# centreborelli/sat-bundleadjust

Hardware: AMD Instinct MI355X
Metric: LM iters/sec at 200 cams x 1M pts x 10M obs (affine, R+T) (higher is better)
Workload: dtype f64; 1 GPU; C4: 200 cams x 1000000 pts x 9998866 obs, affine, correction R+T, 1 fixed camera, seed 1; obs_per_rank0=9998866

## Files before the change

### sat-bundleadjust_amd/csrc/satba_capi.hip

```cpp
#include <hip/hip_runtime.h>

#include <algorithm>
#include <atomic>
#include <chrono>
#include <cmath>
#include <cstdarg>
#include <cstdio>
#include <cstdlib>
#include <cstring>
#include <new>
#include <string>
#include <thread>
#include <vector>

#include "../../include/satba.h"
#include "satba_chol.h"
#include "satba_kernels.h"
#include "satba_layout.h"
#include "satba_lm.h"
#include "satba_lmdev.h"
#include "satba_outliers.h"
#include "satba_triangulate.h"
#include "satba_tracks.h"
#include "satba_ftracks.h"
// ... 51 lines not shown
constexpr int RED_SLOTS = 8, RED_MAX_GRID = 2048, RED_MAX_NV = 4;
struct SchurItems { int2* items = nullptr; SchurItem* desc = nullptr; int n_blocks = 0; };
static_assert(sizeof(SchurItemKey) == sizeof(int2) && offsetof(SchurItemKey, pair) == offsetof(int2, x) && offsetof(SchurItemKey, chunk) == offsetof(int2, y), "uploaded as int2");

struct satba_problem {
    int model = 0, M = 0, N = 0, NP = 0, c_p = 0, n_cam_fix = 0, n_pts_fix = 0, rank = 0, world = 1, f32 = 0, device = 0;
    long long K = 0, n_total = 0;
    int n_c = 0, n = 0, hdr = 0;
    int loss = 0;
    int camc_lds = 0, rpc_lds = 0;
    int cam_sums_lds = 1;
    int lin_rep_shift = 0;
    int deterministic = 0;
    int split_env = -1;
    double *d_fx = nullptr, *d_bbox = nullptr, *d_fxcost = nullptr, *d_fxcost_new = nullptr, *d_fxcost0 = nullptr;
    int *d_fxflag = nullptr, *d_fxe = nullptr;
    bool fxcost_valid = false, fxcost_new_valid = false, fxcost0_valid = false;
    double w_max = 1.0, n_max_cam = 1.0, fx_shrink = 1.0;
    int fx_fallbacks = 0;
    bool scales_by_tail = false;
    bool prep_fused = false;
    struct LmDev* d_lm = nullptr;
    struct LmSummary* h_lm = nullptr;
    struct LmSummary* h_lm_dev = nullptr;
    long long lm_ticks_queued = 0;
    hipStream_t own_stream = nullptr;
    double f_scale = 1.0, lead = 1.0;
    hipStream_t stream = nullptr;
    Layout L;
    int unit_weights = 0;
    double *d_cam_static = nullptr, *d_rpc = nullptr;
    double *d_x = nullptr, *d_xnew = nullptr, *d_camc = nullptr, *d_camc_new = nullptr;
    double *d_scale_inv = nullptr, *d_g = nullptr, *d_gh = nullptr, *d_gn = nullptr, *d_q1 = nullptr, *d_wv = nullptr;
    double *d_U = nullptr, *d_gc = nullptr, *d_V = nullptr, *d_Vinv = nullptr, *d_PV = nullptr, *d_dc = nullptr, *d_dch = nullptr;
    double2 *d_f = nullptr, *d_ftmp = nullptr;
    bool f_valid = false;
    bool prof_lin = false;
    std::vector<hipEvent_t> prof_ev;
    size_t prof_used = 0;
    double* d_Jpm = nullptr;
    double *d_part = nullptr, *d_part3 = nullptr, *d_pair_part = nullptr;
    SchurItems items_chunked;
    SchurItems items_merged;
    double2* d_W = nullptr;
    SchurItems items_w;
    int lin_grid = 0, cm_chunks = 1, cm_chunks_w = 1;
    double* d_red = nullptr;
    unsigned* d_red_cnt = nullptr;
    double* d_stage = nullptr;
    size_t stage_len = 0;
    int* d_fail = nullptr;
    double* d_dinv = nullptr;
    CholWork chol;
    bool s_scaled = false;
    hipStream_t chol_stream = nullptr;
    hipEvent_t ev_fork = nullptr, ev_join = nullptr;
    int* d_arrive = nullptr;
    int* d_pair_cnt = nullptr;
    int* d_dg_cnt = nullptr;
    long long* d_ts = nullptr;
    int msg_epoch = 0;
    double* msg_packed = nullptr;
    bool beside_last = false;
    bool beside_off = false;
    int beside_clean = 0;
    int beside_retry_after = 64;
    int beside_timeouts = 0;
    double* d_scal = nullptr;
    double* d_keep = nullptr;
    bool prepared = false;
    double *d_xb_own = nullptr, *d_xb = nullptr;
    long long xb_len = 0;
    double* h_pin = nullptr;
    bool dir_global = false;
    double* d_dir_tab = nullptr;
    void* h_stage = nullptr;
    size_t h_stage_len = 0;
    struct CopyLane { char* pin = nullptr; hipEvent_t ev[2] = {nullptr, nullptr}; };
    CopyLane lanes[8];
    hipStream_t copy_stream = nullptr;
    bool lanes_ready = false;
    double* d_err_keep = nullptr;
    hipEvent_t ev_err = nullptr;
    double* d_x0 = nullptr;
    bool linearized = false, have_step = false;
    double create_ms[8] = {0, 0, 0, 0, 0, 0, 0, 0};
    std::vector<void*> allocs;

    double* payload() const { return d_xb + hdr; }
    RedBuf red(int slot) const { return RedBuf{d_red + (size_t)slot * RED_MAX_NV * RED_MAX_GRID, d_red_cnt + slot}; }
};
struct PhaseCtx {
    const int* gate = nullptr;
    const double *Delta_dev = nullptr, *coef_dev = nullptr, *lam_force_dev = nullptr, *sub_args_dev = nullptr;
    const int* first_dev = nullptr;
    int fuse_prep = -1;
    bool skip_lin_scales = false;
    bool decide1a_in_trial = false;
    bool decide2_in_trial = false;
};
struct FrontCtx {
    int arrive_epoch = 0;
// ... 264 lines not shown
    CamMajor cm = cam_major(p);
    SATBA_DISPATCH(p, hipLaunchKernelGGL((k_cam_sums<MODEL, NP>), dim3(p->M, p->cm_chunks), dim3(LINC_THREADS), 0, p->stream, a, cm, p->d_f, p->d_part3));
    HIP_TRY(hipGetLastError());
    const int total = p->M * cam_acc_len(p->NP);
    hipLaunchKernelGGL(k_cam_sums_finish, dim3((total + 255) / 256), dim3(256), 0, p->stream, p->M, p->NP, p->cm_chunks, p->d_part3, U, gc, gate);
    HIP_TRY(hipGetLastError());
    return 0;
}

namespace {
struct SchurRoute;
int schur_items_build(satba_problem* p, SchurTable kind, SchurItems* t, long long dg_weight);
int schur_item_tables(satba_problem* p);
template <int MODEL, int NP> int launch_schur(satba_problem* p, const FrontCtx& f, const SchurRoute& r, const ObsArgs& a, double* S, double* rhs);
}
static int launch_schur_kernel(satba_problem* p, const int* gate, const FrontCtx& f, const SchurRoute& r) {
    ObsArgs a = obs_args(p, false, gate);
    double* S = p->payload();
    double* rhs = S + (size_t)p->n_c * p->n_c;
    SATBA_DISPATCH(p, TRY((launch_schur<MODEL, NP>(p, f, r, a, S, rhs))));
    return 0;
}

static int launch_backsub_kernel(satba_problem* p, const int* gate) {
    ObsArgs a = obs_args(p, false, gate);
    a.sh = slice_split(p);
    a.rev = slice_rev(1);
    const int grid = slice_grid(p, BS_THREADS / 64, 2, a.sh);
    const size_t lds = p->model == AFFINE ? dir_table_bytes(p) : table_bytes(p);
    if (p->dir_global) {
        SATBA_DISPATCH(p, if constexpr (MODEL == AFFINE) {
            hipLaunchKernelGGL((k_affine_dir_tab<NP>), dim3(1), dim3(1024), 0, p->stream, a, p->d_dc, (const double*)nullptr, (const double*)nullptr);
            hipLaunchKernelGGL((k_backsub<MODEL, NP, CL, RL, true>), dim3(grid), dim3(BS_THREADS), 0, p->stream, a, p->d_dc, p->d_dch, p->lead,
                               p->d_Vinv, p->d_g, p->d_scale_inv, p->d_gh, p->d_gn, p->red(RB_BS), p->d_xb);
        });
    } else
    SATBA_DISPATCH(p, hipLaunchKernelGGL((k_backsub<MODEL, NP, CL, RL>), dim3(grid), dim3(BS_THREADS), lds, p->stream, a, p->d_dc, p->d_dch, p->lead,
                                         p->d_Vinv, p->d_g, p->d_scale_inv, p->d_gh, p->d_gn, p->red(RB_BS), p->d_xb));
    HIP_TRY(hipGetLastError());
    return 0;
}

static int launch_jvp(satba_problem* p, const int* gate, int nv, const double* q1, const double* q2, double* out, bool pre = false) {
    ObsArgs a = obs_args(p, false, gate);
    a.sh = slice_split(p);
    a.rev = slice_rev(2);
    const int grid = slice_grid(p, JVP_THREADS / 64, 2, a.sh);
    const RedBuf rb = p->red(RB_JVP);
    if (p->dir_global && (nv == 2 || pre)) {
        SATBA_DISPATCH(p, if constexpr (MODEL == AFFINE) {
            hipLaunchKernelGGL((k_affine_dir_tab<NP>), dim3(1), dim3(1024), 0, p->stream, a, q1, nv == 2 ? q2 : nullptr, nv == 2 ? p->d_scale_inv : nullptr);
            if (nv == 1) hipLaunchKernelGGL((k_jvp<MODEL, NP, 1, CL, RL, true, true>), dim3(grid), dim3(JVP_THREADS), 0, p->stream, a, q1, q2, p->d_scale_inv, rb, out);
            else hipLaunchKernelGGL((k_jvp<MODEL, NP, 2, CL, RL, false, true>), dim3(grid), dim3(JVP_THREADS), 0, p->stream, a, q1, q2, p->d_scale_inv, rb, out);
        });
    } else if (nv == 1 && pre) {
        const size_t lds = p->model == AFFINE ? dir_table_bytes(p) : table_bytes(p);
        SATBA_DISPATCH(p, hipLaunchKernelGGL((k_jvp<MODEL, NP, 1, CL, RL, true>), dim3(grid), dim3(JVP_THREADS), lds, p->stream, a, q1, q2, p->d_scale_inv, rb, out));
    } else if (nv == 1) {
        SATBA_DISPATCH(p, hipLaunchKernelGGL((k_jvp<MODEL, NP, 1, CL, RL, false>), dim3(grid), dim3(JVP_THREADS), table_bytes(p), p->stream, a, q1, q2,
                                             p->d_scale_inv, rb, out));
    } else {
        const size_t lds = p->model == AFFINE ? std::max(table_bytes(p), 2 * dir_table_bytes(p)) : table_bytes(p);
        SATBA_DISPATCH(p, hipLaunchKernelGGL((k_jvp<MODEL, NP, 2, CL, RL, false>), dim3(grid), dim3(JVP_THREADS), lds, p->stream, a, q1, q2,
                                             p->d_scale_inv, rb, out));
    }
    HIP_TRY(hipGetLastError());
    return 0;
}

static int dense_solve(satba_problem* p, const int* gate, double* S, double* b, bool cleared = false, bool* unscaled = nullptr) {
    TrsvTail tail;
// ... 284 lines not shown
    if (const char* ss = getenv("SATBA_SPLIT")) p->split_env = atoi(ss);

    int rc = [&]() -> int {
        HIP_TRY(hipSetDevice(p->device));
        HIP_TRY(hipStreamCreateWithFlags(&p->own_stream, hipStreamNonBlocking));
        p->stream = p->own_stream;
        if (p->n_c > CH_NB * CH_MAX_STEPS) return fail(SATBA_E_ARG, "reduced camera system too large for the dense solver");
        cholesky_init();
        TRY(build_layout(p, d));
        const size_t budget = 150 * 1024;
        const size_t camc_b = sizeof(double) * (size_t)p->M * CAMC, rpc_b = sizeof(double) * (size_t)p->M * RPCS;
        while (p->lin_rep_shift < 4 && (p->M << (p->lin_rep_shift + 1)) <= 1024 &&
               cam_sum_bytes(p->NP, (size_t)(p->M << (p->lin_rep_shift + 1))) + camc_b <= 140 * 1024)
            ++p->lin_rep_shift;
        if (const char* rs = getenv("SATBA_LIN_REP")) p->lin_rep_shift = std::min(4, std::max(0, atoi(rs)));
        const size_t acc_b = cam_sum_bytes(p->NP, (size_t)(p->M << p->lin_rep_shift));
        p->cam_sums_lds = (acc_b <= budget && !p->deterministic && !getenv("SATBA_CAM_SUMS") && p->n_max_cam <= (double)FX_MAX_OBS_PER_CAM) ? 1 : 0;
        size_t used = p->cam_sums_lds ? acc_b : 0;
        p->camc_lds = (camc_b <= 48 * 1024 && used + camc_b <= budget && !getenv("SATBA_CAMC_GLOBAL")) ? 1 : 0;
        used += p->camc_lds ? camc_b : 0;
        p->rpc_lds = (p->model == RPC && rpc_b <= 64 * 1024 && used + rpc_b <= budget && !getenv("SATBA_RPC_GLOBAL")) ? 1 : 0;
        p->dir_global = p->model == AFFINE && (2 * dir_table_bytes(p) > budget || getenv("SATBA_DIR_GLOBAL"));
        if (p->dir_global) TRY(dev_alloc(p, &p->d_dir_tab, (size_t)2 * p->M * JVP_ROW));
        SATBA_DISPATCH(p, TRY((raise_lin_limits<MODEL, NP, CL, RL>(p))));

        const size_t n = p->n, Pz = (size_t)std::max(p->L.P, 1) + 64;
        TRY(dev_alloc(p, &p->d_cam_static, (size_t)p->M * p->c_p));
        if (p->model == RPC) TRY(dev_alloc(p, &p->d_rpc, (size_t)p->M * SATBA_RPC_TABLE_LEN));
        TRY(dev_alloc(p, &p->d_x, n)); TRY(dev_alloc(p, &p->d_xnew, n)); TRY(dev_alloc(p, &p->d_scale_inv, n));
        TRY(dev_alloc(p, &p->d_g, n)); TRY(dev_alloc(p, &p->d_gh, n)); TRY(dev_alloc(p, &p->d_gn, n));
        TRY(dev_alloc(p, &p->d_q1, n)); TRY(dev_alloc(p, &p->d_wv, n));
        TRY(dev_alloc(p, &p->d_camc, (size_t)p->M * CAMC)); TRY(dev_alloc(p, &p->d_camc_new, (size_t)p->M * CAMC));
        TRY(dev_alloc(p, &p->d_U, (size_t)p->M * p->NP * p->NP)); TRY(dev_alloc(p, &p->d_gc, p->n_c));
        TRY(dev_alloc(p, &p->d_V, (size_t)6 * p->N)); TRY(dev_alloc(p, &p->d_Vinv, (size_t)6 * p->N));
        TRY(dev_alloc(p, &p->d_PV, (size_t)PV_STRIDE * (p->N + 1)));
        HIP_TRY(hipMemset(p->d_PV + (size_t)PV_STRIDE * p->N, 0, sizeof(double) * PV_STRIDE));
        TRY(dev_alloc(p, &p->d_dc, p->n_c)); TRY(dev_alloc(p, &p->d_dch, p->n_c));
        const size_t Kz = (size_t)std::max<long long>(K, 1) + 64;
        TRY(dev_alloc(p, &p->d_f, Pz)); TRY(dev_alloc(p, &p->d_ftmp, Pz));
        if (p->model == RPC) TRY(dev_alloc(p, &p->d_Jpm, Kz * jrow_stride(p->NP)));
        TRY(dev_alloc(p, &p->d_fail, 1 + CH_MAX_STEPS));
        TRY(dev_alloc(p, &p->d_dinv, (size_t)((p->n_c + CH_NB - 1) / CH_NB) * CH_NB * CH_NB));
        {
            const size_t T = (size_t)(p->n_c + 63) / 64;
            TRY(dev_alloc(p, &p->chol.flags, T * T + 1)); TRY(dev_alloc(p, &p->chol.Linv, T * 4096 + 1)); TRY(dev_alloc(p, &p->chol.Cc, T * T * 64 + 1));
            TRY(dev_alloc(p, &p->chol.ctr, 4));
            HIP_TRY(hipMemset(p->chol.flags, 0, sizeof(int) * (T * T + 1)));
            HIP_TRY(hipMemset(p->chol.ctr, 0, sizeof(int) * 4));
        }
        TRY(dev_alloc(p, &p->d_scal, 8));
        TRY(dev_alloc(p, &p->d_fx, fx_scales_len(p->NP))); TRY(dev_alloc(p, &p->d_fxe, fx_exps_len(p->NP)));
        TRY(dev_alloc(p, &p->d_bbox, 6)); TRY(dev_alloc(p, &p->d_fxflag, 1));
        TRY(dev_alloc(p, &p->d_fxcost, 1)); TRY(dev_alloc(p, &p->d_fxcost_new, 1)); TRY(dev_alloc(p, &p->d_fxcost0, 1));
        HIP_TRY(hipMemset(p->d_bbox, 0, sizeof(double) * 6));
        HIP_TRY(hipMemset(p->d_fxflag, 0, sizeof(int)));
        if (const char* fs = getenv("SATBA_FX_SHRINK")) p->fx_shrink = atof(fs);
        TRY(dev_alloc(p, &p->d_lm, 1));
        HIP_TRY(hipMemset(p->d_lm, 0, sizeof(LmDev)));
        HIP_TRY(hipHostMalloc((void**)&p->h_lm, sizeof(LmSummary) + sizeof(LmDev), hipHostMallocMapped));
        memset(p->h_lm, 0, sizeof(LmSummary) + sizeof(LmDev));
        HIP_TRY(hipHostGetDevicePointer((void**)&p->h_lm_dev, p->h_lm, 0));
        TRY(dev_alloc(p, &p->d_keep, SATBA_KEEP_LEN));
        HIP_TRY(hipMemset(p->d_keep, 0, sizeof(double) * SATBA_KEEP_LEN));
        TRY(dev_alloc(p, &p->d_red, (size_t)RED_SLOTS * RED_MAX_NV * RED_MAX_GRID));
        TRY(dev_alloc(p, &p->d_red_cnt, RED_SLOTS));
        HIP_TRY(hipMemset(p->d_red_cnt, 0, sizeof(unsigned) * RED_SLOTS));
        p->lin_grid = lin_grid_for(p);
        TRY(dev_alloc(p, &p->d_part, (size_t)512 * p->M * cam_sum_len(p->NP)));
        {
            int chunks = 8;
            while (chunks < 64 && (long long)p->M * chunks < 512 && K / ((long long)p->M * (chunks + 8)) >= 4096) chunks += 8;
            while (chunks > 1 && K / ((long long)p->M * chunks) < 256) --chunks;
            int chunks_w = chunks;
            if (chunks >= 8) {
                chunks_w = std::min(64, 2 * chunks);
                while (chunks_w > chunks && K / ((long long)p->M * chunks_w) < 512) chunks_w -= 8;
            }
            if (const char* dc = getenv("SATBA_CM_CHUNKS")) chunks_w = chunks = std::max(1, std::min(256, atoi(dc)));
            p->cm_chunks = chunks; p->cm_chunks_w = chunks_w;
            TRY(dev_alloc(p, &p->d_part3, (size_t)p->M * std::max(64, std::max(chunks, chunks_w)) * (cam_acc_len(p->NP) + p->NP)));
        }
        if (p->L.C > 1) TRY(dev_alloc(p, &p->d_pair_part, (size_t)p->L.C * std::max<long long>(p->L.n_pairs, 1) * p->NP * p->NP));
        TRY(schur_item_tables(p));
        p->stage_len = std::max<size_t>(std::max<size_t>(n, 2 * (size_t)K), (size_t)6 * p->N) + 16;
        TRY(dev_alloc(p, &p->d_stage, p->stage_len));
        p->xb_len = satba_exchange_len(p);
        TRY(dev_alloc(p, &p->d_xb_own, p->xb_len));
        p->d_xb = p->d_xb_own;
        HIP_TRY(hipHostMalloc((void**)&p->h_pin, sizeof(double) * (p->hdr + 64)));
        HIP_TRY(hipMemset(p->d_xb, 0, sizeof(double) * p->xb_len));
        HIP_TRY(hipMemset(p->d_scale_inv, 0, sizeof(double) * n));
        HIP_TRY(hipMemset(p->d_x, 0, sizeof(double) * n));
        HIP_TRY(hipMemset(p->d_xnew, 0, sizeof(double) * n));
        HIP_TRY(hipMemcpy(p->d_cam_static, d->cam_params, sizeof(double) * p->M * p->c_p, hipMemcpyHostToDevice));
        if (p->model == RPC)
            HIP_TRY(hipMemcpy(p->d_rpc, d->rpc_tables, sizeof(double) * p->M * SATBA_RPC_TABLE_LEN, hipMemcpyHostToDevice));
// ... 698 lines not shown
```

### sat-bundleadjust_amd/csrc/satba_kernels.h

```cpp
#pragma once
#include <hip/hip_runtime.h>
#include <stdint.h>

#include "../../include/satba.h"
#include "satba_models.h"

namespace satba {

__host__ __device__ constexpr int cam_acc_len(int np) { return np * (np + 1) / 2 + np; }
__host__ __device__ constexpr int cam_acc_stride(int np) { return cam_acc_len(np) | 1; }
__host__ __device__ constexpr int cam_sum_len(int np) { return 3 * np; }
__host__ __device__ constexpr int cam_sum_stride(int np) { return (3 * np) | 1; }
constexpr int FX_LO_SHIFT = 40;
constexpr long long FX_MAX_OBS_PER_CAM = 1ll << 23;
__host__ __device__ constexpr size_t cam_sum_bytes(int np, size_t rows) { return (rows * cam_sum_stride(np) * 8 + 15) & ~(size_t)15; }
__host__ __device__ constexpr int fx_scales_len(int np) { return 2 * np; }
__host__ __device__ constexpr int fx_exps_len(int np) { return np + 3; }

constexpr int RPCS = 94;
static_assert(RPCS >= 90 && RPCS % 2 == 0 && (RPCS / 2) % 2 == 1, "RPC rows in the LDS: an odd number of 16-byte slots");
constexpr double FX_MAGIC = 6755399441055744.0;
constexpr unsigned long long FX_MAGIC_BITS = 0x4338000000000000ull;
__host__ __device__ constexpr int jrow_stride(int) { return 8; }

// ... 1226 lines not shown
    __syncthreads();
    if (tid < hdr_len) xb[tid] = 0.0;
    if (s_k[2] != 0.0) return;
    if (first_dev) first = *first_dev;
    double s_gh = 0.0, s_xs = 0.0, m_gc = 0.0;
    for (int i = tid; i < n_c; i += 1024) {
        const int cam = i / NP, k = i % NP;
        const double diag = payload[(size_t)cam * NP * NP + k * NP + k], gi = payload[nU + i];
        g[i] = gi;
        m_gc = fmax(m_gc, fabs(gi));
        double si = sqrt(diag);
        if (first) si = (si == 0.0) ? 1.0 : si;
        else si = fmax(si, scale_inv[i]);
        scale_inv[i] = si;
        const double h = gi / si;
        gh[i] = h;
        ghs[i] = h / si;
        s_gh += lead * h * h;
        const double xs = x[i] * si;
        s_xs += lead * xs * xs;
    }
    s_gh = wave_sum(s_gh); s_xs = wave_sum(s_xs); m_gc = wave_max(m_gc);
    if (lane == 0) { s_red[0][wave] = s_gh; s_red[1][wave] = s_xs; s_red[2][wave] = m_gc; }
    __syncthreads();
    if (tid == 0) {
        double a = 0.0, b = 0.0, m = 0.0;
        for (int w = 0; w < 16; ++w) { a += s_red[0][w]; b += s_red[1][w]; m = fmax(m, s_red[2][w]); }
        xb[SATBA_HDR_GH_SQ] = a + s_k[0];
        xb[SATBA_HDR_XS_SQ] = b + s_k[1];
        xb[SATBA_HDR_GC_INF] = lead * m;
    }
}

#ifndef SATBA_BS_THREADS
#define SATBA_BS_THREADS 512
#endif
constexpr int BS_THREADS = SATBA_BS_THREADS;
template <int MODEL, int NP, bool CL, bool RL, bool DG = false>
__global__ __launch_bounds__(BS_THREADS) void k_backsub(ObsArgs a, const double* __restrict__ dc, const double* __restrict__ dch,
                                                        double lead, const double* __restrict__ Vinv, const double* __restrict__ g,
                                                        const double* __restrict__ scale_inv, const double* __restrict__ gh,
                                                        double* __restrict__ gn, RedBuf rb, double* __restrict__ hdr) {
    SATBA_GATE(a.gate);
    extern __shared__ __attribute__((aligned(16))) double s_dyn_bs[];
    const int lane = threadIdx.x & 63;
    constexpr int WAVES = BS_THREADS / 64;
    double sa = 0.0, sb = 0.0, sc = 0.0;
    if (blockIdx.x == 0) {
        for (int i = threadIdx.x; i < a.n_c; i += BS_THREADS) {
            const double v = dch[i], h = gh[i];
            gn[i] = v;
            sa += lead * h * h; sb += lead * h * v; sc += lead * v * v;
        }
    }
    CamTables<CL, RL> T;
    const double* tab = DG ? a.dir_tab : s_dyn_bs;
    if constexpr (MODEL == AFFINE) { if constexpr (!DG) affine_dir_table<NP>(a, dc, s_dyn_bs, BS_THREADS); }
    else T.stage(a, s_dyn_bs, BS_THREADS);
    for_each_slice(a.n_slices << a.sh, WAVES, [&](const int u) {
        const SliceUnit su(a, u, lane);
        const int q = su.q;
        const bool has = q < a.N;
        const int cnt = has ? a.pt_cnt[q] : 0;
        double X = 0.0, Y = 0.0, Z = 0.0, mp = 0.0;
        if (has) {
            const double* px = a.x + a.n_c + 3 * (size_t)q;
            X = px[0]; Y = px[1]; Z = px[2];
            mp = (a.perm[q] >= a.n_pts_fix) ? 1.0 : 0.0;
        }
        double t[3] = {0.0, 0.0, 0.0};
        int pos = su.pos;
        const int io0 = has ? a.ipt_ofs[q] : 0;
        if constexpr (MODEL == AFFINE) {
            constexpr int D = SATBA_CAM_PF;
// ... 20 lines not shown
                    DirRow R;
                    R.load(tab, cam);
                    const double* row = R.v;
                    const double u0 = mp * s2.x * s2.x * (row[0] * X + row[1] * Y + row[2] * Z + row[6]);
                    const double u1 = mp * s2.y * s2.y * (row[3] * X + row[4] * Y + row[5] * Z + row[7]);
#pragma unroll
                    for (int j = 0; j < 3; ++j) t[j] += row[8 + j] * u0 + row[11 + j] * u1;
                }
            }
        } else {
            for (int tt = 0; tt < su.nt; ++tt, pos += su.step) {
                const int k = su.slot(tt);
                if (k < cnt) {
                    const int cam = a.e_cam[pos];
                    ObsEval<MODEL, NP, true> e;
                    e.jac(a, io0 + k, cam, mp, T.cc(cam), T.tab(cam), X, Y, Z);
                    double u0 = 0.0, u1 = 0.0;
#pragma unroll
                    for (int i = 0; i < NP; ++i) {
                        const double d = dc[cam * NP + i];
                        u0 += e.Jc[0][i] * d;
                        u1 += e.Jc[1][i] * d;
                    }
#pragma unroll
                    for (int j = 0; j < 3; ++j) t[j] += e.Jp[0][j] * u0 + e.Jp[1][j] * u1;
                }
            }
        }
        if (su.sh) {
#pragma unroll
            for (int j = 0; j < 3; ++j) t[j] = slice_point_sum(t[j], su.sh);
        }
        if (has && su.g == 0) {
            const double* vi = Vinv + 6 * (size_t)q;
            const size_t ib = (size_t)a.n_c + 3 * (size_t)q;
            const double r0 = g[ib] - t[0], r1 = g[ib + 1] - t[1], r2 = g[ib + 2] - t[2];
            const double d[3] = {vi[0] * r0 + vi[1] * r1 + vi[2] * r2, vi[1] * r0 + vi[3] * r1 + vi[4] * r2,
                                 vi[2] * r0 + vi[4] * r1 + vi[5] * r2};
#pragma unroll
            for (int k = 0; k < 3; ++k) {
                const double v = d[k] * scale_inv[ib + k], h = gh[ib + k];
                gn[ib + k] = v;
                sa += h * h; sb += h * v; sc += v * v;
            }
        }
    }, a.rev);
    double v[3] = {sa, sb, sc};
    double* const dst[3] = {hdr + SATBA_HDR_GRAM_A, hdr + SATBA_HDR_GRAM_B, hdr + SATBA_HDR_GRAM_C};
    grid_sum<3>(v, dst, rb);
}

__global__ __launch_bounds__(256) void k_subspace_vec(int n, int n_c, double lead, double alpha, double s,
                                                      const double* __restrict__ gh, const double* __restrict__ gn,
                                                      double* __restrict__ q1, double* __restrict__ wv, RedBuf rb,
                                                      double* __restrict__ hdr, const double* __restrict__ args_dev, const int* gate) {
    SATBA_GATE(gate);
    if (args_dev) { alpha = args_dev[0]; s = args_dev[1]; }
    double ww = 0.0, wq = 0.0, gw = 0.0;
    for (int i = blockIdx.x * blockDim.x + threadIdx.x; i < n; i += gridDim.x * blockDim.x) {
        const double h = gh[i], q = s * h, w = gn[i] - alpha * h;
        q1[i] = q;
        wv[i] = w;
        const double wgt = (i < n_c) ? lead : 1.0;
        ww += wgt * w * w; wq += wgt * w * q; gw += wgt * h * w;
    }
    double v[3] = {ww, wq, gw};
    double* const dst[3] = {hdr + SATBA_HDR_WW, hdr + SATBA_HDR_WQ1, hdr + SATBA_HDR_GHW};
    grid_sum<3>(v, dst, rb);
// ... 20 lines not shown
```

### sat-bundleadjust_amd/csrc/satba_schur.h

```cpp
#pragma once
#include "satba_kernels.h"

namespace satba {

constexpr int PV_STRIDE = 16;
__device__ inline double schur_lambda(const double* __restrict__ hdr, double Delta, double lam_floor, double* __restrict__ keep, bool write) {
    const double gh_sq = hdr[SATBA_HDR_GH_SQ], jg_sq = hdr[SATBA_HDR_JG_SQ], xs_sq = hdr[SATBA_HDR_XS_SQ];
    if (!(Delta > 0.0)) {
        Delta = sqrt(xs_sq);
        if (Delta == 0.0) Delta = 1.0;
    }
    const double a = 0.5 * jg_sq, b = -gh_sq, ub = Delta / sqrt(gh_sq);
    double best = fmin(0.0, a * ub * ub + b * ub);
    if (a != 0.0) {
        const double ext = -0.5 * b / a;
        if (0.0 < ext && ext < ub) best = fmin(best, a * ext * ext + b * ext);
    }
    double lam = -best / (Delta * Delta);
    if (!(lam >= lam_floor)) lam = lam_floor;
    if (write) {
        keep[SATBA_KEEP_GINF] = fmax(keep[SATBA_KEEP_GINF], hdr[SATBA_HDR_GC_INF]);
        keep[SATBA_KEEP_GH_SQ] = gh_sq; keep[SATBA_KEEP_JG_SQ] = jg_sq; keep[SATBA_KEEP_XS_SQ] = xs_sq;
        keep[SATBA_KEEP_LAM] = lam;
        keep[SATBA_KEEP_DELTA] = Delta;
    }
    return lam;
}

#ifndef SATBA_VINV_THREADS
#define SATBA_VINV_THREADS 256
#endif
constexpr int VINV_THREADS = SATBA_VINV_THREADS;
__global__ __launch_bounds__(VINV_THREADS) void k_vinv(int N, double lam, const double* __restrict__ hdr_auto, double Delta, double lam_floor,
                                                       double* __restrict__ keep, const double* __restrict__ V,
                                                       const double* __restrict__ scale_inv_p, double* __restrict__ Vinv,
                                                       const double* __restrict__ xp, const double* __restrict__ gp, double* __restrict__ PV,
                                                       const int* __restrict__ perm, int n_pts_fix, const double* __restrict__ Delta_dev,
                                                       const double* __restrict__ lam_force, const int* gate, const int* __restrict__ w_fix = nullptr) {
    SATBA_GATE(gate);
    if (Delta_dev) Delta = *Delta_dev;
    if (lam_force && *lam_force > 0.0) {
        hdr_auto = nullptr;
        lam = *lam_force;
        if (blockIdx.x == 0 && threadIdx.x == 0) keep[SATBA_KEEP_LAM] = lam;
    }
    __shared__ double2 s_t[VINV_THREADS / 64][64 * 9];
    const int lane = threadIdx.x & 63, wave = threadIdx.x >> 6;
    const int p0 = (blockIdx.x * (VINV_THREADS / 64) + wave) * 64;
    if (p0 >= N) return;
    const int p = min(p0 + lane, N - 1);
    if (hdr_auto) lam = schur_lambda(hdr_auto, Delta, lam_floor, keep, p0 + lane == 0);
    const double2* v2 = reinterpret_cast<const double2*>(V + 6 * (size_t)p);
    const double2 va = v2[0], vb = v2[1], vc = v2[2];
    const double* s = scale_inv_p + 3 * (size_t)p;
    const double a = va.x + lam * s[0] * s[0], b = va.y, c = vb.x;
    const double d = vb.y + lam * s[1] * s[1], e = vc.x, f = vc.y + lam * s[2] * s[2];
    const double c00 = d * f - e * e, c01 = c * e - b * f, c02 = b * e - c * d;
    const double idet = 1.0 / (a * c00 + b * c01 + c * c02);
    const double o0 = c00 * idet, o1 = c01 * idet, o2 = c02 * idet;
    const double o3 = (a * f - c * c) * idet, o4 = (b * c - a * e) * idet, o5 = (a * d - b * b) * idet;
    const double x0 = xp[3 * (size_t)p], x1 = xp[3 * (size_t)p + 1], x2 = xp[3 * (size_t)p + 2];
    const double g0 = gp[3 * (size_t)p], g1 = gp[3 * (size_t)p + 1], g2 = gp[3 * (size_t)p + 2];
    const double mp = (perm[p] >= n_pts_fix) ? 1.0 : 0.0;
    double2* t = s_t[wave];
    const int n_here = min(64, N - p0);
    t[3 * lane] = make_double2(o0, o1); t[3 * lane + 1] = make_double2(o2, o3); t[3 * lane + 2] = make_double2(o4, o5);
    asm volatile("" ::: "memory");
    __builtin_amdgcn_wave_barrier();
    {
        double2* out = reinterpret_cast<double2*>(Vinv + 6 * (size_t)p0);
#pragma unroll
        for (int k = 0; k < 3; ++k) {
            const int g = 64 * k + lane;
            const double2 v = t[g];
            if (g < 3 * n_here) out[g] = v;
        }
    }
    asm volatile("" ::: "memory");
    __builtin_amdgcn_wave_barrier();
    static_assert(PV_STRIDE == 16, "records are eight 16-byte pieces");
    double2* row = t + 9 * lane;
    row[0] = make_double2(x0, x1); row[1] = make_double2(x2, mp * o0); row[2] = make_double2(mp * o1, mp * o2);
    row[3] = make_double2(mp * o3, mp * o4); row[4] = make_double2(mp * o5, g0); row[5] = make_double2(g1, g2);
    asm volatile("" ::: "memory");
    __builtin_amdgcn_wave_barrier();
    if (w_fix) {
        double2* out = reinterpret_cast<double2*>(PV);
#pragma unroll
        for (int k = 0; k < 8; ++k) {
            const int g = 64 * k + lane, r = g >> 3, q = g & 7;
            const double2 v = t[9 * r + (q < 6 ? q : 0)];
            const int at = w_fix[min(p0 + r, N - 1)];
            if (q < 6 && r < n_here) out[(size_t)at + q] = v;
        }
        return;
    }
    {
        double2* out = reinterpret_cast<double2*>(PV + PV_STRIDE * (size_t)p0);
#pragma unroll
        for (int k = 0; k < 8; ++k) {
            const int g = 64 * k + lane, r = g >> 3, q = g & 7;
            const double2 v = t[9 * r + (q < 6 ? q : 0)];
            if (q < 6 && r < n_here) out[g] = v;
        }
    }
}

struct SchurItem {
    long long lo, hi;
    int i, j;
    int pair, chunk;
};
// ... 212 lines not shown
        asm volatile("s_waitcnt vmcnt(0)" ::: "memory");
        if (lane == 0) __hip_atomic_fetch_add(s.arrive + (size_t)SCHUR_ARRIVE_STRIDE * i, 1, __ATOMIC_RELAXED, __HIP_MEMORY_SCOPE_AGENT);
        return;
    }
#pragma unroll
    for (int ps = 0; ps < NPS; ++ps) {
        if (ev[ps] >= NB2) continue;
        if (s.n_chunks > 1) part[ev[ps]] = total[ps];
        else if (!s.arrive) *out(ev[ps]) = total[ps];
        else __hip_atomic_store(out(ev[ps]), total[ps], __ATOMIC_RELAXED, __HIP_MEMORY_SCOPE_AGENT);
    }
    if (s.arrive && s.n_chunks == 1) {
        asm volatile("s_waitcnt vmcnt(0)" ::: "memory");
        if (lane == 0) __hip_atomic_fetch_add(s.arrive + (size_t)SCHUR_ARRIVE_STRIDE * i, 1, __ATOMIC_RELAXED, __HIP_MEMORY_SCOPE_AGENT);
    }
}

template <int MODEL, int NP, bool UNITW>
__device__ __forceinline__ void schur_pairs_body(const ObsArgs& a, const SchurArgs& s, double* __restrict__ S, const unsigned bidx, double2* s_coop, unsigned (*s_idx)[3 * 64]) {
    const int lane = threadIdx.x & 63, wave = threadIdx.x >> 6;
    const long long n_pairs = (long long)a.M * (a.M - 1) / 2;
    const SchurItem* dp = s.desc + (bidx * 4u + (unsigned)wave);
    const int i = __builtin_amdgcn_readfirstlane(dp->i);
    if (i < 0) return;
    const int j = __builtin_amdgcn_readfirstlane(dp->j);
    const int chunk = __builtin_amdgcn_readfirstlane(dp->chunk);
    const long long pair = __builtin_amdgcn_readfirstlane(dp->pair);
    if constexpr (!UNITW && MODEL != RPC) {
        if (i == j) {
            constexpr int CU = cam_acc_len(NP), CPAD = CU <= 16 ? 16 : 32;
            double dacc[CU];
#pragma unroll
            for (int k = 0; k < CU; ++k) dacc[k] = 0.0;
            schur_diag_walk<MODEL, NP, 64>(a, s.PV, s.cm_rec, s.cm_sc, 1, s.zero_fix, i, (int)dp->lo, (int)dp->hi, lane,
                                           reinterpret_cast<double2*>(reinterpret_cast<char*>(s_coop) + wave * (64 * 112)), dacc);
            const double cam_mask = i < a.n_cam_fix ? 0.0 : 1.0;
            if constexpr (CU > 32) {
#pragma unroll
                for (int o = 0; o < CU; o += 64) {
                    double flat[64];
#pragma unroll
                    for (int e = 0; e < 64; ++e) flat[e] = (o + e < CU) ? dacc[o + e] : 0.0;
                    const double total = cam_mask * wave_reduce_scatter<64>(flat, lane, 32);
                    const int e = o + rs_index<64>(lane);
                    double* const mine = s.dg_part + ((size_t)i * s.n_dg + chunk) * CU + e;
                    if (e < CU) {
                        if (!s.arrive) *mine = total;
                        else __hip_atomic_store(mine, total, __ATOMIC_RELAXED, __HIP_MEMORY_SCOPE_AGENT);
                    }
                }
                if (!s.arrive) return;
            } else {
            double flat[CPAD];
#pragma unroll
            for (int e = 0; e < CPAD; ++e) flat[e] = (e < CU) ? dacc[e] : 0.0;
            const double total = cam_mask * wave_reduce_scatter<CPAD>(flat, lane, 32);
            const int e = rs_index<CPAD>(lane);
            double* const mine = s.dg_part + ((size_t)i * s.n_dg + chunk) * CU + e;
            const bool writer = (lane & (64 / CPAD - 1)) == 0 && e < CU;
            if (!s.arrive) {
                if (writer) *mine = total;
                return;
            }
            if (writer) __hip_atomic_store(mine, total, __ATOMIC_RELAXED, __HIP_MEMORY_SCOPE_AGENT);
            }
            asm volatile("s_waitcnt vmcnt(0)" ::: "memory");
            if (bidx == 0 && threadIdx.x == 0)
// ... 122 lines not shown
            rpc_jac_from_d<NP>(cci, X, Y, Z, Di, Jci, Jpi);
            rpc_jac_from_d<NP>(ccj, X, Y, Z, Dj, Jcj, Jpj);
        } else {
            double u, v;
            project<MODEL, NP, true>(cci, nullptr, X, Y, Z, false, u, v, Jci, Jpi);
            project<MODEL, NP, true>(ccj, nullptr, X, Y, Z, false, u, v, Jcj, Jpj);
        }
        double A[2][3];
#pragma unroll
        for (int r = 0; r < 2; ++r) {
            A[r][0] = Jpi[r][0] * v00 + Jpi[r][1] * v01 + Jpi[r][2] * v02;
            A[r][1] = Jpi[r][0] * v01 + Jpi[r][1] * v11 + Jpi[r][2] * v12;
            A[r][2] = Jpi[r][0] * v02 + Jpi[r][1] * v12 + Jpi[r][2] * v22;
        }
        double m00 = A[0][0] * Jpj[0][0] + A[0][1] * Jpj[0][1] + A[0][2] * Jpj[0][2];
        double m01 = A[0][0] * Jpj[1][0] + A[0][1] * Jpj[1][1] + A[0][2] * Jpj[1][2];
        double m10 = A[1][0] * Jpj[0][0] + A[1][1] * Jpj[0][1] + A[1][2] * Jpj[0][2];
        double m11 = A[1][0] * Jpj[1][0] + A[1][1] * Jpj[1][1] + A[1][2] * Jpj[1][2];
        if constexpr (MODEL != RPC && !UNITW) {
            const double ax = scl_i.x * scl_i.x, ay = scl_i.y * scl_i.y;
            const double bx = scl_j.x * scl_j.x, by = scl_j.y * scl_j.y;
            m00 *= ax * bx; m01 *= ax * by; m10 *= ay * bx; m11 *= ay * by;
        }
#pragma unroll
        for (int q = 0; q < NP; ++q) {
            const double y0 = m00 * Jcj[0][q] + m01 * Jcj[1][q];
            const double y1 = m10 * Jcj[0][q] + m11 * Jcj[1][q];
#pragma unroll
            for (int r = 0; r < NP; ++r) acc[r][q] = fma(-Jci[0][r], y0, fma(-Jci[1][r], y1, acc[r][q]));
        }
    };

    {
        const long long lo = dp->lo, hi = dp->hi;
        constexpr bool POS = !UNITW || MODEL == RPC;
        constexpr bool SCL = !UNITW && MODEL != RPC;
        const int n_it = (int)((hi - lo + 63) >> 6);
        if (n_it > 0) {
            const long long last = hi - 1;
            auto ld = [&](const int* arr, long long k) { return __builtin_nontemporal_load(arr + (k < last ? k : last)); };
            auto ldp = [&](long long k) { const int v = ld(SCL ? s.pair_rec : s.pair_pts, k); return (k < hi) ? v : (SCL ? s.zero_fix : a.N); };
            auto ldk = [&](long long k) { const int v = ld(s.pair_kk, k); return (k < hi) ? v : 0x00010001; };
            constexpr int NPC = SCL ? 7 : 5;
            struct Coop { double2 c0, c1, c2, c3, c4, c5, c6; };
            int rsrc[NPC];
            const double2* psrc[NPC];
            unsigned pcv[NPC];
            int kind[NPC];
#pragma unroll
            for (int t = 0; t < NPC; ++t) {
                const int g = 64 * t + lane, pc = g % NPC;
                rsrc[t] = g / NPC;
                pcv[t] = (unsigned)pc;
                kind[t] = 64 * (pc < 5 ? 0 : pc - 4) + g / NPC;
                psrc[t] = pc < 5 ? s.PV + pc : reinterpret_cast<const double2*>(a.sc);
            }
            unsigned* sidx = s_idx[wave];
            auto coop_load = [&](int p, int pi, int pj) {
                Coop o;
                if constexpr (SCL) {
                    asm volatile("" ::: "memory");
                    sidx[lane] = (unsigned)p; sidx[64 + lane] = (unsigned)p - ((unsigned)pi & 0xffffu); sidx[128 + lane] = (unsigned)p - ((unsigned)pi >> 16);
                    asm volatile("" ::: "memory");
                    __builtin_amdgcn_wave_barrier();
                    const unsigned o0 = sidx[kind[0]], o1 = sidx[kind[1]], o2 = sidx[kind[2]], o3 = sidx[kind[3]], o4 = sidx[kind[4]],
                                   o5 = sidx[kind[NPC - 2]], o6 = sidx[kind[NPC - 1]];
                    asm volatile("" ::: "memory");
// ... 282 lines not shown
                const double ag0 = sx * (A[0][0] * r4.y + A[0][1] * r5.x + A[0][2] * r5.y);
                const double ag1 = sy * (A[1][0] * r4.y + A[1][1] * r5.x + A[1][2] * r5.y);
                int k = 0;
#pragma unroll
                for (int r = 0; r < NP; ++r) {
                    const double y0 = m00 * Jc[0][r] + m01 * Jc[1][r];
                    const double y1 = m01 * Jc[0][r] + m11 * Jc[1][r];
#pragma unroll
                    for (int q = r; q < NP; ++q) {
                        acc[k] -= Jc[0][q] * y0 + Jc[1][q] * y1;
                        acc[k] += ux * Jc[0][r] * Jc[0][q] + uy * Jc[1][r] * Jc[1][q];
                        ++k;
                    }
                }
#pragma unroll
                for (int r = 0; r < NP; ++r) acc[k++] -= Jc[0][r] * ag0 + Jc[1][r] * ag1;
            }
            __builtin_amdgcn_sched_barrier(0);
        }
    }
}

template <int MODEL, int NP>
__device__ __forceinline__ void schur_diag_body(const ObsArgs& a, const CamMajor& c, const SchurArgs& s, double* __restrict__ part, const int L, const int M,
                                                const int n_chunks, double2* s_coop, double (*s_red)[cam_acc_len(NP)]) {
    constexpr int CU = cam_acc_len(NP);
    int cam = L % M, chunk = L / M;
    if (s.diag_xcd) {
        const int x = L & 7, q = L >> 3;
        cam = q % M; chunk = (q / M) * 8 + x;
    }
    const int b = c.cam_ofs[cam], e = c.cam_ofs[cam + 1];
    const long long len = e - b;
    const int lo = b + (int)(len * chunk / n_chunks), hi = b + (int)(len * (chunk + 1) / n_chunks);
    const int lane = threadIdx.x & 63, wave = threadIdx.x >> 6;
    double acc[CU];
#pragma unroll
    for (int k = 0; k < CU; ++k) acc[k] = 0.0;
    schur_diag_walk<MODEL, NP, LINC_THREADS>(a, s.PV, c.pt, c.io, s.wmode ? 1 : PV_STRIDE / 2, s.wmode ? s.zero_fix : (PV_STRIDE / 2) * a.N, cam, lo, hi,
                                             (int)threadIdx.x, s_coop + wave * (64 * 7), acc);
    if (cam < a.n_cam_fix) {
#pragma unroll
        for (int k = 0; k < CU; ++k) acc[k] = 0.0;
    }
#pragma unroll
    for (int k = 0; k < CU; ++k) {
        const double t = wave_sum(acc[k]);
        if (lane == 0) s_red[wave][k] = t;
    }
    __syncthreads();
    if (threadIdx.x < CU) {
        double t = 0.0;
        for (int wv = 0; wv < LINC_THREADS / 64; ++wv) t += s_red[wv][threadIdx.x];
        part[((size_t)cam * n_chunks + chunk) * CU + threadIdx.x] = t;
    }
}
template <int MODEL, int NP>
__global__ __launch_bounds__(LINC_THREADS) void k_schur_diag(ObsArgs a, CamMajor c, SchurArgs s, double* __restrict__ part) {
    SATBA_GATE(a.gate);
    __shared__ double2 s_coop[(LINC_THREADS / 64) * 64 * 7];
    __shared__ double s_red[LINC_THREADS / 64][cam_acc_len(NP)];
    schur_diag_body<MODEL, NP>(a, c, s, part, (int)(blockIdx.y * gridDim.x + blockIdx.x), (int)gridDim.x, (int)gridDim.y, s_coop, s_red);
}
static_assert(LINC_THREADS == 256, "k_schur_both: both bodies run 256 threads");
template <int MODEL, int NP, bool UNITW>
__global__ __launch_bounds__(256) SATBA_PAIRS_WAVES_ATTR(MODEL, NP, UNITW) void k_schur_both(ObsArgs a, CamMajor c, SchurArgs s, double* __restrict__ part, double* __restrict__ S,
                                                                                      int n_diag, int n_diag_pad, int M, int n_chunks) {
    SATBA_GATE(a.gate);
    __shared__ double2 s_coop[4 * 64 * 7];
    __shared__ unsigned s_idx[4][3 * 64];
    __shared__ double s_red[4][cam_acc_len(NP)];
    if ((int)blockIdx.x < n_diag_pad) {
        if ((int)blockIdx.x < n_diag) schur_diag_body<MODEL, NP>(a, c, s, part, (int)blockIdx.x, M, n_chunks, s_coop, s_red);
        return;
    }
    schur_pairs_body<MODEL, NP, UNITW>(a, s, S, blockIdx.x - (unsigned)n_diag_pad, s_coop, s_idx);
}
// ... 44 lines not shown
```

### sat-bundleadjust_amd/csrc/satba_schur_api.inc

```
extern "C++" {
namespace {

int schur_items_build(satba_problem* p, SchurTable kind, SchurItems* t, long long dg_weight) {
    const bool w = kind == SCHUR_ITEMS_WEIGHTED;
    const std::vector<SchurItemKey> table = schur_item_order(kind, p->M, p->L.C, w ? p->L.dg_spc : 0, dg_weight);
    t->n_blocks = (int)(table.size() / 4);
    TRY(dev_alloc(p, &t->items, table.size()));
    HIP_TRY(hipMemcpy(t->items, table.data(), sizeof(int2) * table.size(), hipMemcpyHostToDevice));
    TRY(dev_alloc(p, &t->desc, table.size()));
    hipLaunchKernelGGL(k_schur_item_desc, dim3((unsigned)((table.size() + 255) / 256)), dim3(256), 0, p->stream, (long long)table.size(), t->items,
                       p->L.pair_ij, p->L.pair_ofs, p->L.C, t->desc, w ? p->L.dg_ofs : (const int*)nullptr, w ? p->L.n_dg : 1);
    HIP_TRY(hipGetLastError());
    return 0;
}
bool schur_merge_enough(const satba_problem* p) {
    const char* mg = getenv("SATBA_SCHUR_MERGE");
    return p->L.n_pairs >= 8192 || (mg && atoi(mg) != 0);
}
int schur_item_tables(satba_problem* p) {
    TRY(schur_items_build(p, SCHUR_ITEMS_CHUNKED, &p->items_chunked, 0));
    const char* mg = getenv("SATBA_SCHUR_MERGE");
    if (p->L.C > 1 && schur_merge_enough(p) && !(mg && atoi(mg) == 0)) TRY(schur_items_build(p, SCHUR_ITEMS_MERGED, &p->items_merged, 0));
    return 0;
}
// ... 65 lines not shown
        hipLaunchKernelGGL(k_schur_finish, dim3((unsigned)(r.nb_diag + (outs + 255) / 256)), dim3(256), 0, p->stream, p->M, NP, p->n_c, r.finish_dchunks, p->d_part3,
                           f.lam, f.lam_dev, p->lead, p->d_gc, p->d_scale_inv, S, rhs, p->d_xb, (int)p->hdr, r.nb_diag, r.finish_red_chunks,
                           p->L.pair_ij, p->d_pair_part, a.gate, r.finish_scale ? p->d_dch : (double*)nullptr, r.finish_scale ? p->d_fail : (int*)nullptr,
                           r.finish_scale ? 1 + CH_MAX_STEPS : 0);
        p->s_scaled = r.finish_scale;
    };
    if (!r.dg_in_pairs && !r.both) hipLaunchKernelGGL((k_schur_diag<MODEL, NP>), dim3(p->M, r.dchunks), dim3(LINC_THREADS), 0, p->stream, a, cm, s, p->d_part3);
    if (r.finish_first) finish();
    if (r.pairs_run) {
        const dim3 igrid((unsigned)r.items->n_blocks);
        if (r.both) {
            const int n_diag = p->M * r.dchunks, n_diag_pad = (n_diag + 7) & ~7;
            const dim3 bgrid(igrid.x + (unsigned)n_diag_pad);
            if (r.unit) hipLaunchKernelGGL((k_schur_both<MODEL, NP, true>), bgrid, dim3(256), 0, p->stream, a, cm, s, p->d_part3, S, n_diag, n_diag_pad, p->M, r.dchunks);
            else hipLaunchKernelGGL((k_schur_both<MODEL, NP, false>), bgrid, dim3(256), 0, p->stream, a, cm, s, p->d_part3, S, n_diag, n_diag_pad, p->M, r.dchunks);
        }
        else if (r.unit) hipLaunchKernelGGL((k_schur_pairs<MODEL, NP, true>), igrid, dim3(256), 0, p->stream, a, s, S);
        else hipLaunchKernelGGL((k_schur_pairs<MODEL, NP, false>), igrid, dim3(256), 0, p->stream, a, s, S);
        HIP_TRY(hipGetLastError());
    }
    if (!r.finish_first) finish();
    HIP_TRY(hipGetLastError());
    return 0;
}

int schur_impl(satba_problem* p, const PhaseCtx& c, FrontCtx f, double lam, bool automatic, double Delta, double lam_floor) {
    Range range_("satba:schur");
    if (!p->linearized || (automatic && !p->prepared)) return fail(SATBA_E_STATE, automatic ? "schur_auto before prepare" : "schur before linearize");
    if (automatic) p->prepared = false;
    const SchurRoute r = schur_route(p, f);
    if (p->N > 0) {
        const bool w = r.weighted;
        hipLaunchKernelGGL(k_vinv, dim3((p->N + VINV_THREADS - 1) / VINV_THREADS), dim3(VINV_THREADS), 0, p->stream, p->N, lam, automatic ? p->d_xb : nullptr, Delta, lam_floor,
                           p->d_keep, p->d_V, p->d_scale_inv + p->n_c, p->d_Vinv, p->d_x + p->n_c, p->d_g + p->n_c, w ? reinterpret_cast<double*>(p->d_W) : p->d_PV,
                           p->L.perm, p->n_pts_fix, automatic ? c.Delta_dev : nullptr, automatic ? c.lam_force_dev : nullptr, c.gate,
                           w ? p->L.w_fix : (const int*)nullptr);
    } else if (automatic) {
        hipLaunchKernelGGL(k_lambda, dim3(1), dim3(1), 0, p->stream, p->d_xb, Delta, lam_floor, p->d_keep, c.Delta_dev, c.lam_force_dev, c.gate);
    }
    HIP_TRY(hipGetLastError());
    if (!r.pairs_run) HIP_TRY(hipMemsetAsync(p->d_xb + p->hdr, 0, sizeof(double) * ((size_t)p->n_c * p->n_c + p->n_c), p->stream));
    f.lam = lam; f.lam_dev = automatic ? p->d_keep + SATBA_KEEP_LAM : nullptr;
    return launch_schur_kernel(p, c.gate, f, r);
}

void beside_disable(satba_problem* p) {
    if (p->beside_timeouts > 0) p->beside_retry_after = std::min(p->beside_retry_after * 2, 1 << 20);
    p->beside_off = true; p->beside_clean = 0; ++p->beside_timeouts;
    (void)hipStreamSynchronize(p->chol_stream);
    (void)hipMemsetAsync(p->d_arrive, 0, sizeof(int) * (size_t)(p->M + 2) * SCHUR_ARRIVE_STRIDE, p->stream);
    (void)hipMemsetAsync(p->d_pair_cnt, 0, sizeof(int) * (size_t)std::max<long long>(p->L.n_pairs, 1), p->stream);
    (void)hipMemsetAsync(p->d_dg_cnt, 0, sizeof(int) * (size_t)p->M, p->stream);
}
bool beside_timed_out(satba_problem* p, const double* h) {
    if (!p->beside_last || !(h[SATBA_HDR_CHOL_FAIL] >= SATBA_CHOL_BESIDE_WAIT)) return false;
    beside_disable(p);
    return true;
}
int chol_front_streams(satba_problem* p) {
    if (p->chol_stream) return 0;
    int least = 0, greatest = 0, mine = 0;
    HIP_TRY(hipDeviceGetStreamPriorityRange(&least, &greatest));
    HIP_TRY(hipStreamGetPriority(p->stream, &mine));
    HIP_TRY(hipStreamCreateWithPriority(&p->chol_stream, hipStreamNonBlocking, mine != greatest ? greatest : least));
    HIP_TRY(hipEventCreateWithFlags(&p->ev_fork, hipEventDisableTiming));
    HIP_TRY(hipEventCreateWithFlags(&p->ev_join, hipEventDisableTiming));
    TRY(dev_alloc(p, &p->d_arrive, (size_t)(p->M + 2) * SCHUR_ARRIVE_STRIDE));
// ... 163 lines not shown
```

Before: 892.8 LM iters/sec.

## Recompute point block inverse in backsub and skip fixed-camera Schur walks

The Vinv buffer is removed. k_vinv no longer writes 6 doubles per point, and records only the lambda it used. Backsub reads V and recomputes the 3x3 damped inverse per point, trading a global write and read for a small amount of arithmetic. Separately, the Schur diagonal and pair walks now take an empty range for fixed cameras instead of walking their observations and zeroing the result. This relies on those contributions being masked anyway.

```diff
diff --git a/sat-bundleadjust_amd/csrc/satba_capi.hip b/sat-bundleadjust_amd/csrc/satba_capi.hip
--- a/sat-bundleadjust_amd/csrc/satba_capi.hip
+++ b/sat-bundleadjust_amd/csrc/satba_capi.hip
@@ -107,7 +107,7 @@
     double *d_cam_static = nullptr, *d_rpc = nullptr;
     double *d_x = nullptr, *d_xnew = nullptr, *d_camc = nullptr, *d_camc_new = nullptr;
     double *d_scale_inv = nullptr, *d_g = nullptr, *d_gh = nullptr, *d_gn = nullptr, *d_q1 = nullptr, *d_wv = nullptr;
-    double *d_U = nullptr, *d_gc = nullptr, *d_V = nullptr, *d_Vinv = nullptr, *d_PV = nullptr, *d_dc = nullptr, *d_dch = nullptr;
+    double *d_U = nullptr, *d_gc = nullptr, *d_V = nullptr, *d_PV = nullptr, *d_dc = nullptr, *d_dch = nullptr;
     double2 *d_f = nullptr, *d_ftmp = nullptr;
     bool f_valid = false;
     bool prof_lin = false;
@@ -143,6 +143,7 @@
     int beside_timeouts = 0;
     double* d_scal = nullptr;
     double* d_keep = nullptr;
+    double* d_lam_used = nullptr;
     bool prepared = false;
     double *d_xb_own = nullptr, *d_xb = nullptr;
     long long xb_len = 0;
@@ -473,11 +474,11 @@
         SATBA_DISPATCH(p, if constexpr (MODEL == AFFINE) {
             hipLaunchKernelGGL((k_affine_dir_tab<NP>), dim3(1), dim3(1024), 0, p->stream, a, p->d_dc, (const double*)nullptr, (const double*)nullptr);
             hipLaunchKernelGGL((k_backsub<MODEL, NP, CL, RL, true>), dim3(grid), dim3(BS_THREADS), 0, p->stream, a, p->d_dc, p->d_dch, p->lead,
-                               p->d_Vinv, p->d_g, p->d_scale_inv, p->d_gh, p->d_gn, p->red(RB_BS), p->d_xb);
+                               p->d_V, p->d_lam_used, p->d_g, p->d_scale_inv, p->d_gh, p->d_gn, p->red(RB_BS), p->d_xb);
         });
     } else
     SATBA_DISPATCH(p, hipLaunchKernelGGL((k_backsub<MODEL, NP, CL, RL>), dim3(grid), dim3(BS_THREADS), lds, p->stream, a, p->d_dc, p->d_dch, p->lead,
-                                         p->d_Vinv, p->d_g, p->d_scale_inv, p->d_gh, p->d_gn, p->red(RB_BS), p->d_xb));
+                                         p->d_V, p->d_lam_used, p->d_g, p->d_scale_inv, p->d_gh, p->d_gn, p->red(RB_BS), p->d_xb));
     HIP_TRY(hipGetLastError());
     return 0;
 }
@@ -828,7 +829,7 @@
         TRY(dev_alloc(p, &p->d_q1, n)); TRY(dev_alloc(p, &p->d_wv, n));
         TRY(dev_alloc(p, &p->d_camc, (size_t)p->M * CAMC)); TRY(dev_alloc(p, &p->d_camc_new, (size_t)p->M * CAMC));
         TRY(dev_alloc(p, &p->d_U, (size_t)p->M * p->NP * p->NP)); TRY(dev_alloc(p, &p->d_gc, p->n_c));
-        TRY(dev_alloc(p, &p->d_V, (size_t)6 * p->N)); TRY(dev_alloc(p, &p->d_Vinv, (size_t)6 * p->N));
+        TRY(dev_alloc(p, &p->d_V, (size_t)6 * p->N));
         TRY(dev_alloc(p, &p->d_PV, (size_t)PV_STRIDE * (p->N + 1)));
         HIP_TRY(hipMemset(p->d_PV + (size_t)PV_STRIDE * p->N, 0, sizeof(double) * PV_STRIDE));
         TRY(dev_alloc(p, &p->d_dc, p->n_c)); TRY(dev_alloc(p, &p->d_dch, p->n_c));
@@ -858,6 +859,8 @@
         HIP_TRY(hipHostGetDevicePointer((void**)&p->h_lm_dev, p->h_lm, 0));
         TRY(dev_alloc(p, &p->d_keep, SATBA_KEEP_LEN));
         HIP_TRY(hipMemset(p->d_keep, 0, sizeof(double) * SATBA_KEEP_LEN));
+        TRY(dev_alloc(p, &p->d_lam_used, 1));
+        HIP_TRY(hipMemset(p->d_lam_used, 0, sizeof(double)));
         TRY(dev_alloc(p, &p->d_red, (size_t)RED_SLOTS * RED_MAX_NV * RED_MAX_GRID));
         TRY(dev_alloc(p, &p->d_red_cnt, RED_SLOTS));
         HIP_TRY(hipMemset(p->d_red_cnt, 0, sizeof(unsigned) * RED_SLOTS));
diff --git a/sat-bundleadjust_amd/csrc/satba_kernels.h b/sat-bundleadjust_amd/csrc/satba_kernels.h
--- a/sat-bundleadjust_amd/csrc/satba_kernels.h
+++ b/sat-bundleadjust_amd/csrc/satba_kernels.h
@@ -1282,14 +1282,24 @@
     }
 }
 
+__device__ __forceinline__ void point_block_inverse(double v0, double v1, double v2, double v3, double v4, double v5, double lam, double s0,
+                                                    double s1, double s2, double (&o)[6]) {
+    const double a = v0 + lam * s0 * s0, b = v1, c = v2;
+    const double d = v3 + lam * s1 * s1, e = v4, f = v5 + lam * s2 * s2;
+    const double c00 = d * f - e * e, c01 = c * e - b * f, c02 = b * e - c * d;
+    const double idet = 1.0 / (a * c00 + b * c01 + c * c02);
+    o[0] = c00 * idet; o[1] = c01 * idet; o[2] = c02 * idet;
+    o[3] = (a * f - c * c) * idet; o[4] = (b * c - a * e) * idet; o[5] = (a * d - b * b) * idet;
+}
+
 #ifndef SATBA_BS_THREADS
 #define SATBA_BS_THREADS 512
 #endif
 constexpr int BS_THREADS = SATBA_BS_THREADS;
 template <int MODEL, int NP, bool CL, bool RL, bool DG = false>
 __global__ __launch_bounds__(BS_THREADS) void k_backsub(ObsArgs a, const double* __restrict__ dc, const double* __restrict__ dch,
-                                                        double lead, const double* __restrict__ Vinv, const double* __restrict__ g,
-                                                        const double* __restrict__ scale_inv, const double* __restrict__ gh,
+                                                        double lead, const double* __restrict__ V, const double* __restrict__ lam_used,
+                                                        const double* __restrict__ g, const double* __restrict__ scale_inv, const double* __restrict__ gh,
                                                         double* __restrict__ gn, RedBuf rb, double* __restrict__ hdr) {
     SATBA_GATE(a.gate);
     extern __shared__ __attribute__((aligned(16))) double s_dyn_bs[];
@@ -1376,8 +1386,11 @@
             for (int j = 0; j < 3; ++j) t[j] = slice_point_sum(t[j], su.sh);
         }
         if (has && su.g == 0) {
-            const double* vi = Vinv + 6 * (size_t)q;
             const size_t ib = (size_t)a.n_c + 3 * (size_t)q;
+            const double2* v2 = reinterpret_cast<const double2*>(V + 6 * (size_t)q);
+            const double2 va = v2[0], vb = v2[1], vc = v2[2];
+            double vi[6];
+            point_block_inverse(va.x, va.y, vb.x, vb.y, vc.x, vc.y, *lam_used, scale_inv[ib], scale_inv[ib + 1], scale_inv[ib + 2], vi);
             const double r0 = g[ib] - t[0], r1 = g[ib + 1] - t[1], r2 = g[ib + 2] - t[2];
             const double d[3] = {vi[0] * r0 + vi[1] * r1 + vi[2] * r2, vi[1] * r0 + vi[3] * r1 + vi[4] * r2,
                                  vi[2] * r0 + vi[4] * r1 + vi[5] * r2};
diff --git a/sat-bundleadjust_amd/csrc/satba_schur.h b/sat-bundleadjust_amd/csrc/satba_schur.h
--- a/sat-bundleadjust_amd/csrc/satba_schur.h
+++ b/sat-bundleadjust_amd/csrc/satba_schur.h
@@ -33,7 +33,7 @@
 constexpr int VINV_THREADS = SATBA_VINV_THREADS;
 __global__ __launch_bounds__(VINV_THREADS) void k_vinv(int N, double lam, const double* __restrict__ hdr_auto, double Delta, double lam_floor,
                                                        double* __restrict__ keep, const double* __restrict__ V,
-                                                       const double* __restrict__ scale_inv_p, double* __restrict__ Vinv,
+                                                       const double* __restrict__ scale_inv_p, double* __restrict__ lam_used,
                                                        const double* __restrict__ xp, const double* __restrict__ gp, double* __restrict__ PV,
                                                        const int* __restrict__ perm, int n_pts_fix, const double* __restrict__ Delta_dev,
                                                        const double* __restrict__ lam_force, const int* gate, const int* __restrict__ w_fix = nullptr) {
@@ -50,34 +50,18 @@
     if (p0 >= N) return;
     const int p = min(p0 + lane, N - 1);
     if (hdr_auto) lam = schur_lambda(hdr_auto, Delta, lam_floor, keep, p0 + lane == 0);
+    if (p0 + lane == 0) *lam_used = lam;
     const double2* v2 = reinterpret_cast<const double2*>(V + 6 * (size_t)p);
     const double2 va = v2[0], vb = v2[1], vc = v2[2];
     const double* s = scale_inv_p + 3 * (size_t)p;
-    const double a = va.x + lam * s[0] * s[0], b = va.y, c = vb.x;
-    const double d = vb.y + lam * s[1] * s[1], e = vc.x, f = vc.y + lam * s[2] * s[2];
-    const double c00 = d * f - e * e, c01 = c * e - b * f, c02 = b * e - c * d;
-    const double idet = 1.0 / (a * c00 + b * c01 + c * c02);
-    const double o0 = c00 * idet, o1 = c01 * idet, o2 = c02 * idet;
-    const double o3 = (a * f - c * c) * idet, o4 = (b * c - a * e) * idet, o5 = (a * d - b * b) * idet;
+    double o[6];
+    point_block_inverse(va.x, va.y, vb.x, vb.y, vc.x, vc.y, lam, s[0], s[1], s[2], o);
+    const double o0 = o[0], o1 = o[1], o2 = o[2], o3 = o[3], o4 = o[4], o5 = o[5];
     const double x0 = xp[3 * (size_t)p], x1 = xp[3 * (size_t)p + 1], x2 = xp[3 * (size_t)p + 2];
     const double g0 = gp[3 * (size_t)p], g1 = gp[3 * (size_t)p + 1], g2 = gp[3 * (size_t)p + 2];
     const double mp = (perm[p] >= n_pts_fix) ? 1.0 : 0.0;
     double2* t = s_t[wave];
     const int n_here = min(64, N - p0);
-    t[3 * lane] = make_double2(o0, o1); t[3 * lane + 1] = make_double2(o2, o3); t[3 * lane + 2] = make_double2(o4, o5);
-    asm volatile("" ::: "memory");
-    __builtin_amdgcn_wave_barrier();
-    {
-        double2* out = reinterpret_cast<double2*>(Vinv + 6 * (size_t)p0);
-#pragma unroll
-        for (int k = 0; k < 3; ++k) {
-            const int g = 64 * k + lane;
-            const double2 v = t[g];
-            if (g < 3 * n_here) out[g] = v;
-        }
-    }
-    asm volatile("" ::: "memory");
-    __builtin_amdgcn_wave_barrier();
     static_assert(PV_STRIDE == 16, "records are eight 16-byte pieces");
     double2* row = t + 9 * lane;
     row[0] = make_double2(x0, x1); row[1] = make_double2(x2, mp * o0); row[2] = make_double2(mp * o1, mp * o2);
@@ -356,7 +340,7 @@
             double dacc[CU];
 #pragma unroll
             for (int k = 0; k < CU; ++k) dacc[k] = 0.0;
-            schur_diag_walk<MODEL, NP, 64>(a, s.PV, s.cm_rec, s.cm_sc, 1, s.zero_fix, i, (int)dp->lo, (int)dp->hi, lane,
+            schur_diag_walk<MODEL, NP, 64>(a, s.PV, s.cm_rec, s.cm_sc, 1, s.zero_fix, i, (int)dp->lo, i < a.n_cam_fix ? (int)dp->lo : (int)dp->hi, lane,
                                            reinterpret_cast<double2*>(reinterpret_cast<char*>(s_coop) + wave * (64 * 112)), dacc);
             const double cam_mask = i < a.n_cam_fix ? 0.0 : 1.0;
             if constexpr (CU > 32) {
@@ -545,7 +529,8 @@
     };
 
     {
-        const long long lo = dp->lo, hi = dp->hi;
+        const bool cam_fixed = i < a.n_cam_fix || j < a.n_cam_fix;
+        const long long lo = dp->lo, hi = cam_fixed ? lo : dp->hi;
         constexpr bool POS = !UNITW || MODEL == RPC;
         constexpr bool SCL = !UNITW && MODEL != RPC;
         const int n_it = (int)((hi - lo + 63) >> 6);
@@ -894,17 +879,14 @@
     }
     const int b = c.cam_ofs[cam], e = c.cam_ofs[cam + 1];
     const long long len = e - b;
-    const int lo = b + (int)(len * chunk / n_chunks), hi = b + (int)(len * (chunk + 1) / n_chunks);
+    const int lo = b + (int)(len * chunk / n_chunks);
+    const int hi = cam < a.n_cam_fix ? lo : b + (int)(len * (chunk + 1) / n_chunks);
     const int lane = threadIdx.x & 63, wave = threadIdx.x >> 6;
     double acc[CU];
 #pragma unroll
     for (int k = 0; k < CU; ++k) acc[k] = 0.0;
     schur_diag_walk<MODEL, NP, LINC_THREADS>(a, s.PV, c.pt, c.io, s.wmode ? 1 : PV_STRIDE / 2, s.wmode ? s.zero_fix : (PV_STRIDE / 2) * a.N, cam, lo, hi,
                                              (int)threadIdx.x, s_coop + wave * (64 * 7), acc);
-    if (cam < a.n_cam_fix) {
-#pragma unroll
-        for (int k = 0; k < CU; ++k) acc[k] = 0.0;
-    }
 #pragma unroll
     for (int k = 0; k < CU; ++k) {
         const double t = wave_sum(acc[k]);
diff --git a/sat-bundleadjust_amd/csrc/satba_schur_api.inc b/sat-bundleadjust_amd/csrc/satba_schur_api.inc
--- a/sat-bundleadjust_amd/csrc/satba_schur_api.inc
+++ b/sat-bundleadjust_amd/csrc/satba_schur_api.inc
@@ -121,7 +121,7 @@
     if (p->N > 0) {
         const bool w = r.weighted;
         hipLaunchKernelGGL(k_vinv, dim3((p->N + VINV_THREADS - 1) / VINV_THREADS), dim3(VINV_THREADS), 0, p->stream, p->N, lam, automatic ? p->d_xb : nullptr, Delta, lam_floor,
-                           p->d_keep, p->d_V, p->d_scale_inv + p->n_c, p->d_Vinv, p->d_x + p->n_c, p->d_g + p->n_c, w ? reinterpret_cast<double*>(p->d_W) : p->d_PV,
+                           p->d_keep, p->d_V, p->d_scale_inv + p->n_c, p->d_lam_used, p->d_x + p->n_c, p->d_g + p->n_c, w ? reinterpret_cast<double*>(p->d_W) : p->d_PV,
                            p->L.perm, p->n_pts_fix, automatic ? c.Delta_dev : nullptr, automatic ? c.lam_force_dev : nullptr, c.gate,
                            w ? p->L.w_fix : (const int*)nullptr);
     } else if (automatic) {
```

After: 902.2 LM iters/sec (median of 6 runs). +1.1%, better.
